# openMVG/openMVG

Hardware: AMD Instinct MI355X
Metric: descriptor pairs/s (brute-force L2 2-NN + ratio matching) (higher is better)
Workload: dtype i8 (int32 accumulate); 1 GPU; 1000 images x 2000 SIFT-like uint8x128 descriptors, exhaustive pairs (499500 image pairs, 499500 on rank 0), ratio 0.8; parallelism=pair-sharded x1, no collective

## Files before the change

### openmvg_amd/csrc/mvgx_match.hip

```cpp
#include <hip/hip_runtime.h>

#include <algorithm>
#include <atomic>
#include <climits>
#include <condition_variable>
#include <cstdint>
#include <cstdlib>
#include <cstring>
#include <functional>
#include <mutex>
#include <string>
#include <thread>
#include <vector>

#include "mvgx_buffers.h"
#include "mvgx_common.h"
#include "mvgx_match_batch.h"

namespace {

using mvgx::DevBuf;
using mvgx::PinnedBuf;
using mvgx::set_error;

// ... 703 lines not shown
  stage_window_glds_asm(buf, gtiles, grconst, wave, lane);
#endif
}

__device__ __forceinline__ void fold_window16(const int (&TW)[4], int (&TP)[4], int& Q1, int& Q2, int& Qg, int win) {
  const int v = max(max3i(TW[0], TW[1], TW[2]), TW[3]);
#pragma unroll
  for (int c = 0; c < 4; ++c) TP[c] = max(TP[c], TW[c]);
  Qg = v > Q1 ? win : Qg;
  Q2 = med3i(Q1, v, Q2);
  asm volatile("" : "+v"(Q1));
  Q1 = max(Q1, v);
}

struct UnitBlock { uint32_t pair, tileJ0, row0, nJ; };
__device__ __forceinline__ UnitBlock unit_block(const uint4& a, const uint4& b, uint32_t n) {
  const bool inA = n < b.z;
  return UnitBlock{inA ? a.x : b.x, inA ? a.y : b.y, (inA ? a.z + n : n - b.z) * 16u, inA ? a.w : b.w};
}

#define MVGX_FINISH16_MED3(N, INB, VALID)                                                                                                 \
  {                                                                                                                                       \
    int p1 = kNegInit, p2 = kNegInit, pc = 0;                                                \
    _Pragma("unroll") for (int c = 0; c < 4; ++c) {                                                                                       \
      const int v = TP[N][c];                                                                                                             \
      pc = v > p1 ? c : pc;                                                                                                               \
      p2 = med3i(p1, v, p2);                                                                                                              \
      p1 = max(p1, v);                                                                                                                    \
    }                                                                                                                                     \
                          \
    int W1 = 2 * p1 - par, V2 = max(2 * p2 - par, 2 * Q2[N] - par);                                                                       \
    int code = (4 * (pc >> 1) + 2 * (g4 >> 1) + (pc & 1)) | (par << 3) | (Qg[N] << 4);    \
                                                  \
    _Pragma("unroll") for (int x = 16; x <= 32; x <<= 1) {                                                                                \
      const int o1 = __shfl_xor(W1, x), o2 = __shfl_xor(V2, x), oc = __shfl_xor(code, x);                                                 \
      const bool mine = W1 > o1;                                                                                                          \
      V2 = mine ? max(V2, o1) : max(o2, W1);                                                                                              \
      code = mine ? code : oc;                                                                                                            \
      W1 = mine ? W1 : o1;                                                                                                                \
    }                                                                                                                                     \
    const UnitBlock ub = unit_block(wa, wb, (uint32_t)(N));                  \
    const uint32_t q = ub.row0 + (uint32_t)(lane & 15);                                                                                   \
    if (lane < 16 && (INB)) {                                                                                                             \
      const int nq = qn[N];                                                                                                               \
      const int d0 = nq - W1, d1ub = nq - V2;                                                                                             \
      const bool cand = (VALID) && (__int2float_rn(d0) < __fmul_rn(p.ratio_sq, __int2float_rn(d1ub)));                                    \
      const size_t o = (size_t)ub.pair * p.qstride + q;                                                                                   \
      p.best[o] = cand ? (uint32_t)code : kNoMatch;                                                                                       \
      if (cand) p.cd[o] = make_int2(d0, d1ub);                                                                                            \
    }                                                                                                                                     \
  }

__global__ __launch_bounds__(256, 2) void l2_filter16_kernel(MatchParams p) {
  extern __shared__ __attribute__((aligned(16))) char smem[];

  const int lane = threadIdx.x & 63;
  const int wave = __builtin_amdgcn_readfirstlane(threadIdx.x >> 6);
  const int g4 = lane >> 4, par = g4 & 1;

  const uint32_t w = xcd_remap(blockIdx.x, gridDim.x);
  const uint4* rec = p.work8 + (size_t)kRecQuads * w;
  const uint4 wsh = rec[0], wa = rec[1 + 2 * wave], wb = rec[2 + 2 * wave];
  const uint32_t tileI0 = wsh.x;
  const int ntI = (int)wsh.y;
  const int nwin = (ntI + kWinTiles - 1) / kWinTiles;

  const int lane_chunk = ((lane >> 5) * 64 + ((lane >> 4) & 1) * 32 + (lane & 15)) * 16;
  v4i b[kNB16][2];
  {
#pragma unroll
    for (int n = 0; n < kNB16; ++n) {
      const UnitBlock ub = unit_block(wa, wb, (uint32_t)n);
      const int8_t* qsrc = p.qtiles + ((size_t)(ub.tileJ0 + (ub.row0 >> 5)) * kTileBytes + ((ub.row0 >> 4) & 1u) * 256u) + lane_chunk;
#pragma unroll
      for (int ks = 0; ks < 2; ++ks) b[n][ks] = *reinterpret_cast<const v4i*>(qsrc + ks * 2048);
    }
  }

  const int8_t* gI = p.tiles + (size_t)tileI0 * kTileBytes;
  const int* gC = p.cinit + (size_t)tileI0 * kTileRows;

  int qn[kNB16];
#pragma unroll
  for (int n = 0; n < kNB16; ++n) {
    const UnitBlock ub = unit_block(wa, wb, (uint32_t)n);
    const uint32_t q = ub.row0 + (uint32_t)(lane & 15);
    qn[n] = (lane < 16 && q < ub.nJ) ? p.qtnorm[(size_t)ub.tileJ0 * kTileRows + q] : 0;
  }

  int TP[kNB16][4];
  int TW[kNB16][4];
  int Q1[kNB16], Q2[kNB16], Qg[kNB16];
#pragma unroll
  for (int n = 0; n < kNB16; ++n) {
#pragma unroll
    for (int c = 0; c < 4; ++c) TP[n][c] = kNegInit;
    Q1[n] = kNegInit; Q2[n] = kNegInit; Qg[n] = 0;
  }

  const unsigned voff16 = (unsigned)(lane * 16 + wave * 1024), voff4 = (unsigned)(lane * 4 + wave * 256);
  stage_window16(smem, gI, gC, voff16, voff4, wave, lane);
#pragma unroll
  for (int n = 0; n < kNB16; ++n) {
#pragma unroll
    for (int ks = 0; ks < 2; ++ks) asm volatile("" : "+v"(b[n][ks]));
    asm volatile("" : "+v"(qn[n]));
  }

  for (int win = 0; win < nwin; ++win) {
    asm volatile("s_waitcnt vmcnt(0)" ::: "memory");
    __syncthreads();
    char* buf = smem + (win & 1) * kStageBytes;
    char* nbuf = smem + ((win + 1) & 1) * kStageBytes;
    if (win + 1 < nwin)
      stage_window16(nbuf, gI + (size_t)(win + 1) * kWinTiles * kTileBytes, gC + (win + 1) * kWinRows, voff16, voff4, wave, lane);

    const int nt = min(kWinTiles, ntI - win * kWinTiles);
    const char* wb = buf + lane_chunk;
    const char* wc = buf + kWinTiles * kTileBytes + g4 * 16;
    v4i accA[4], accB[4];

#define MVGX_BLOCK16(A, CV, AN, CN, BLK, LD, NEXT_OFF, NEXT_COFF, EPI_B, MIX_B, EPI_A)                      \
  {                                                                                                         \
    MVGX_GROUP16(accA, 0, A, CV)                                                                            \
    if (LD) {                                                                                               \
      AN[0] = *reinterpret_cast<const v4i*>(wb + (NEXT_OFF));                                               \
      AN[1] = *reinterpret_cast<const v4i*>(wb + (NEXT_OFF) + 2048);                                        \
    }                                                                                                       \
    EPI_B(accB, 4, 1 - (BLK))                                                                               \
    MIX_B((LD) ? 2 : 0)                                                                                     \
    MVGX_GROUP16(accB, 4, A, CV)                                                                            \
    if (LD) CN = *reinterpret_cast<const v4i*>(wc + (NEXT_COFF));                                           \
    EPI_A(accA, 0, BLK)                                                                                     \
    MVGX_MIX16((LD) ? 1 : 0)                                                                                \
  }
#define MVGX_TILE16(T)                                                                                                                       \
  MVGX_BLOCK16(a0, c0, a1, c1, 0, true, (T) * kTileBytes + 256, (T) * (kTileRows * 4) + 64, MVGX_EPI16, MVGX_MIX16, MVGX_EPI16)              \
  MVGX_BLOCK16(a1, c1, a0, c0, 1, true, ((T) + 1) * kTileBytes, ((T) + 1) * (kTileRows * 4), MVGX_EPI16, MVGX_MIX16, MVGX_EPI16)                \
  MVGX_TILE16_END
#define MVGX_TILE16_END __builtin_amdgcn_sched_barrier(0);
    v4i a0[2], a1[2], c0, c1;
    a0[0] = *reinterpret_cast<const v4i*>(wb);
    a0[1] = *reinterpret_cast<const v4i*>(wb + 2048);
    c0 = *reinterpret_cast<const v4i*>(wc);
    __builtin_amdgcn_s_setprio(3);
    if (nt == kWinTiles) {
      MVGX_BLOCK16(a0, c0, a1, c1, 0, true, 256, 64, MVGX_EPI16_NONE, MVGX_MIX16_NOEPI, MVGX_EPI16_FIRST)
      MVGX_BLOCK16(a1, c1, a0, c0, 1, true, kTileBytes, kTileRows * 4, MVGX_EPI16_FIRST, MVGX_MIX16, MVGX_EPI16_FIRST)
      MVGX_TILE16_END
      MVGX_BLOCK16(a0, c0, a1, c1, 0, true, kTileBytes + 256, kTileRows * 4 + 64, MVGX_EPI16_FIRST, MVGX_MIX16, MVGX_EPI16)
      MVGX_BLOCK16(a1, c1, a0, c0, 1, true, 2 * kTileBytes, 2 * (kTileRows * 4), MVGX_EPI16, MVGX_MIX16, MVGX_EPI16)
      MVGX_TILE16_END
      MVGX_TILE16(2) MVGX_TILE16(3) MVGX_TILE16(4) MVGX_TILE16(5) MVGX_TILE16(6)
      MVGX_BLOCK16(a0, c0, a1, c1, 0, true, 7 * kTileBytes + 256, 7 * (kTileRows * 4) + 64, MVGX_EPI16, MVGX_MIX16, MVGX_EPI16)
      MVGX_BLOCK16(a1, c1, a0, c0, 1, false, 0, 0, MVGX_EPI16, MVGX_MIX16, MVGX_EPI16)
    } else {
#pragma unroll
      for (int n = 4; n < kNB16; ++n) { TW[n][2] = kNegInit; TW[n][3] = kNegInit; }
      const int t1 = min(1, nt - 1);
      MVGX_BLOCK16(a0, c0, a1, c1, 0, true, 256, 64, MVGX_EPI16_NONE, MVGX_MIX16_NOEPI, MVGX_EPI16_FIRST)
      MVGX_BLOCK16(a1, c1, a0, c0, 1, true, t1 * kTileBytes, t1 * (kTileRows * 4), MVGX_EPI16_FIRST, MVGX_MIX16, MVGX_EPI16_FIRST)
      for (int t = 1; t < nt; ++t) {
        const int tn = min(t + 1, nt - 1);
        MVGX_BLOCK16(a0, c0, a1, c1, 0, true, t * kTileBytes + 256, t * (kTileRows * 4) + 64, MVGX_EPI16, MVGX_MIX16, MVGX_EPI16)
        MVGX_BLOCK16(a1, c1, a0, c0, 1, true, tn * kTileBytes, tn * (kTileRows * 4), MVGX_EPI16, MVGX_MIX16, MVGX_EPI16)
      }
    }
    MVGX_EPI16(accB, 4, 1)
    __builtin_amdgcn_s_setprio(0);
#undef MVGX_TILE16
#undef MVGX_TILE16_END
#undef MVGX_BLOCK16
#pragma unroll
    for (int n = 0; n < kNB16; ++n) fold_window16(TW[n], TP[n], Q1[n], Q2[n], Qg[n], win);
  }

#pragma unroll
  for (int n = 0; n < kNB16; ++n) MVGX_FINISH16_MED3(n, q < ub.nJ, true)
}

constexpr int kNQh = 2;
constexpr int kNBh = 2 * kNQh;
constexpr int kBlockQTilesH = kWaves * kNQh;
__global__ __launch_bounds__(256, 3) void l2_filter16h_kernel(MatchParams p) {
  extern __shared__ __attribute__((aligned(16))) char smem[];

  const int lane = threadIdx.x & 63;
  const int wave = __builtin_amdgcn_readfirstlane(threadIdx.x >> 6);
  const int g4 = lane >> 4, par = g4 & 1;

  const uint32_t w = xcd_remap(blockIdx.x, gridDim.x);
  const uint4 wr0 = p.work8h[2 * (size_t)w], wr1 = p.work8h[2 * (size_t)w + 1];
  const uint32_t pair = wr0.x;
  const uint32_t tileI0 = wr0.z, tileJ0 = wr0.w;
  const uint32_t ntJpad = wr1.y;
  const int ntI = (int)wr1.x;
  const int nhalf = (ntI + kHalfTiles - 1) / kHalfTiles;
  const uint32_t qt0 = wr0.y + (uint32_t)wave * kNQh;

  const int lane_chunk = ((lane >> 5) * 64 + ((lane >> 4) & 1) * 32 + (lane & 15)) * 16;
  v4i b[kNBh][2];
  {
    const int8_t* qsrc = p.tiles + (size_t)(tileJ0 + qt0) * kTileBytes + lane_chunk;
#pragma unroll
    for (int n = 0; n < kNBh; ++n)
#pragma unroll
      for (int ks = 0; ks < 2; ++ks) b[n][ks] = *reinterpret_cast<const v4i*>(qsrc + (n >> 1) * kTileBytes + (n & 1) * 256 + ks * 2048);
  }
  const int8_t* gI = p.tiles + (size_t)tileI0 * kTileBytes;
  const int* gC = p.cinit + (size_t)tileI0 * kTileRows;

  uint32_t qperm[kNBh];
  int qn[kNBh];
#pragma unroll
  for (int n = 0; n < kNBh; ++n) {
    const bool inb = lane < 16 && qt0 + (uint32_t)(n >> 1) < ntJpad;
    const size_t qs = (size_t)tileJ0 * kTileRows + (qt0 + (uint32_t)(n >> 1)) * kTileRows + (uint32_t)(n & 1) * 16 + (uint32_t)(lane & 15);
    qperm[n] = inb ? p.perm[qs] : kNoMatch;
    qn[n] = inb ? p.qnorm[qs] : 0;
  }

  int TP[kNBh][4], TW[kNBh][4], Q1[kNBh], Q2[kNBh], Qg[kNBh];
#pragma unroll
  for (int n = 0; n < kNBh; ++n) {
#pragma unroll
    for (int c = 0; c < 4; ++c) { TP[n][c] = kNegInit; TW[n][c] = kNegInit; }
    Q1[n] = kNegInit; Q2[n] = kNegInit; Qg[n] = 0;
  }

  stage_half_glds_asm(smem, gI, gC, wave, lane);
#pragma unroll
  for (int n = 0; n < kNBh; ++n) {
#pragma unroll
    for (int ks = 0; ks < 2; ++ks) asm volatile("" : "+v"(b[n][ks]));
    asm volatile("" : "+v"(qperm[n]), "+v"(qn[n]));
  }

  for (int hw = 0; hw < nhalf; ++hw) {
    asm volatile("s_waitcnt vmcnt(0)" ::: "memory");
    __syncthreads();
    char* buf = smem + (hw & 1) * kHalfStageBytes;
    char* nbuf = smem + ((hw + 1) & 1) * kHalfStageBytes;
    if (hw + 1 < nhalf)
      stage_half_glds_asm(nbuf, gI + (size_t)(hw + 1) * kHalfTiles * kTileBytes, gC + (hw + 1) * kHalfTiles * kTileRows, wave, lane);

    const int nt = min(kHalfTiles, ntI - hw * kHalfTiles);
    const char* wb = buf + lane_chunk;
    const char* wc = buf + kHalfTiles * kTileBytes + g4 * 16;
    v4i accA[4], accB[4];
#pragma unroll
    for (int i = 0; i < 4; ++i) accB[i] = v4i{kNegInit, kNegInit, kNegInit, kNegInit};
    v4i a0[2], a1[2], c0, c1;
    a0[0] = *reinterpret_cast<const v4i*>(wb);
    a0[1] = *reinterpret_cast<const v4i*>(wb + 2048);
    c0 = *reinterpret_cast<const v4i*>(wc);
    for (int t = 0; t < nt; ++t) {
      const int tn = min(t + 1, nt - 1);
      MVGX_GROUP16(accA, 0, a0, c0)
      a1[0] = *reinterpret_cast<const v4i*>(wb + t * kTileBytes + 256);
      a1[1] = *reinterpret_cast<const v4i*>(wb + t * kTileBytes + 256 + 2048);
      c1 = *reinterpret_cast<const v4i*>(wc + t * (kTileRows * 4) + 64);
      MVGX_EPI16(accB, 0, 1)
      MVGX_MIX16(3)
      MVGX_GROUP16(accB, 0, a1, c1)
      a0[0] = *reinterpret_cast<const v4i*>(wb + tn * kTileBytes);
      a0[1] = *reinterpret_cast<const v4i*>(wb + tn * kTileBytes + 2048);
      c0 = *reinterpret_cast<const v4i*>(wc + tn * (kTileRows * 4));
      MVGX_EPI16(accA, 0, 0)
      MVGX_MIX16(3)
    }
    MVGX_EPI16(accB, 0, 1)
    if ((hw & 1) || hw + 1 == nhalf) {
#pragma unroll
      for (int n = 0; n < kNBh; ++n) fold_window<4>(TW[n], TP[n], Q1[n], Q2[n], Qg[n], hw >> 1);
    }
  }

#pragma unroll
  for (int n = 0; n < kNBh; ++n) MVGX_FINISH16(n, qt0 + (uint32_t)(n >> 1) < ntJpad, qperm[n] != kNoMatch)
}
#undef MVGX_FINISH16
#undef MVGX_GROUP16
#undef MVGX_EPI16
#undef MVGX_MIX16

__device__ __forceinline__ int sum8_dpp(int v) {
  v += __builtin_amdgcn_update_dpp(0, v, 0xB1, 0xF, 0xF, true);
  v += __builtin_amdgcn_update_dpp(0, v, 0x4E, 0xF, 0xF, true);
  v += __builtin_amdgcn_update_dpp(0, v, 0x141, 0xF, 0xF, true);
  return v;
}
__device__ __forceinline__ int min16_dpp(int v) {
  v = min(v, __builtin_amdgcn_update_dpp(INT_MAX, v, 0xB1, 0xF, 0xF, false));
  v = min(v, __builtin_amdgcn_update_dpp(INT_MAX, v, 0x4E, 0xF, 0xF, false));
  v = min(v, __builtin_amdgcn_update_dpp(INT_MAX, v, 0x141, 0xF, 0xF, false));
  v = min(v, __builtin_amdgcn_update_dpp(INT_MAX, v, 0x140, 0xF, 0xF, false));
  return v;
}

template <bool kWaveUnits>
__global__ __launch_bounds__(256) void l2_verify_kernel(MatchParams p) {
  const int lane = threadIdx.x & 63;
  const int wave = threadIdx.x >> 6;
  uint32_t pair, qt0, I, tileI0, tileJ0, qend;
  uint4 wa = make_uint4(0, 0, 0, 0), wb = wa;
  const uint8_t *rowsJA = nullptr, *rowsJB = nullptr;
  if constexpr (kWaveUnits) {
    const uint4* rec = p.work8 + (size_t)kRecQuads * blockIdx.x;
    const int wu = __builtin_amdgcn_readfirstlane(wave);
    wa = rec[1 + 2 * wu]; wb = rec[2 + 2 * wu];
    tileI0 = rec[0].x;
    const uint2 ijA = p.pairs[wa.x], ijB = p.pairs[wb.x];
    I = ijA.x;
    rowsJA = p.rows_u8 + p.img_row_off[ijA.y] * kDim;
    rowsJB = p.rows_u8 + p.img_row_off[ijB.y] * kDim;
    pair = 0; qt0 = 0; tileJ0 = 0; qend = 0;
  } else {
    const uint2 wk = p.work[blockIdx.x];
    const uint2 ij = p.pairs[wk.x];
    pair = wk.x; qt0 = wk.y + (uint32_t)wave * kNQ;
    I = ij.x;
    tileI0 = p.img_tile_off[I]; tileJ0 = p.img_tile_off[ij.y];
    qend = (p.img_tile_off[ij.y + 1] - tileJ0) * kTileRows;
  }
  const uint32_t nEvenI = p.img_neven[I], nOddI = p.img_n[I] - nEvenI;
  const int l16 = lane & 15, sub = lane >> 4;
  uint32_t accepted = 0, acceptedB = 0;
  for (int part = 0; part < 2; ++part) {
    const uint32_t q0 = qt0 * kTileRows + (uint32_t)part * 64;
    uint32_t q = q0 + lane, qpair = pair;
    bool inb = q < qend;
    if constexpr (kWaveUnits) {
      const UnitBlock ub = unit_block(wa, wb, (uint32_t)(part * 4 + sub));
      q = ub.row0 + (uint32_t)l16; qpair = ub.pair; inb = q < ub.nJ;
    }
    const uint32_t code = inb ? p.best[(size_t)qpair * p.qstride + q] : kNoMatch;
    unsigned long long todo = __ballot(code != kNoMatch);
    while (todo) {
      unsigned long long m = todo;
      for (int i = 0; i < sub; ++i) m &= m - 1;
      const bool active = m != 0;
      const int src = active ? __builtin_ctzll(m) : 0;
      for (int i = 0; i < 4; ++i) todo &= todo - 1;
      const uint32_t cc = (uint32_t)__shfl((int)code, src);
      uint32_t qs = q0 + (uint32_t)src, cpair = pair;
      bool inA = true;
      const uint8_t* rowsJ = nullptr;
      if constexpr (kWaveUnits) {
        const uint32_t cb = (uint32_t)(part * 4 + (src >> 4));
        const UnitBlock ub = unit_block(wa, wb, cb);
        qs = ub.row0 + (uint32_t)(src & 15); cpair = ub.pair; inA = cb < wb.z;
        rowsJ = inA ? rowsJA : rowsJB;
      }
      const int s1 = cc & 7, hw = (cc >> 3) & 1, g1 = (int)(cc >> 4);
      const int piece = l16 & 7, rsel = l16 >> 3;
      const int mrow = slot_row(2 * s1 + rsel, hw);
      const size_t slot0 = (size_t)tileI0 * kTileRows + (active ? (size_t)g1 * kWinTiles * kTileRows + mrow : 0);
      const size_t slotQ = (size_t)tileJ0 * kTileRows + (active ? qs : 0);
      const size_t o = (size_t)cpair * p.qstride + (active ? qs : 0);
      const uint32_t tt = (uint32_t)g1 * kWinTiles + (uint32_t)piece;
      const size_t slotI = active ? slot0 + (size_t)piece * kTileRows : slot0;
      const bool valid = active && (tt * 16u + (uint32_t)(2 * s1 + rsel)) < (hw ? nOddI : nEvenI);
      int4 va[8];
#pragma unroll
      for (int c = 0; c < 8; ++c)
        va[c] = *reinterpret_cast<const int4*>(p.rows_slot + (slot0 + (active ? (size_t)c * kTileRows : 0)) * kDim + piece * 16);
      int4 vb;
      if constexpr (kWaveUnits) {
        vb = *reinterpret_cast<const int4*>(rowsJ + (size_t)(active ? qs : 0) * kDim + piece * 16);
        vb.x ^= (int)0x80808080u; vb.y ^= (int)0x80808080u; vb.z ^= (int)0x80808080u; vb.w ^= (int)0x80808080u;
      } else {
        vb = *reinterpret_cast<const int4*>(p.rows_slot + slotQ * kDim + piece * 16);
      }
      const int2 f = p.cd[o];
      const int f_d0 = f.x, f_d1 = f.y;
      int nb = __builtin_amdgcn_sdot4(vb.x, vb.x, 0, false);
      nb = __builtin_amdgcn_sdot4(vb.y, vb.y, nb, false);
      nb = __builtin_amdgcn_sdot4(vb.z, vb.z, nb, false);
      nb = __builtin_amdgcn_sdot4(vb.w, vb.w, nb, false);
      nb = sum8_dpp(nb);
      int dot = 0, na = 0;
#pragma unroll
      for (int c = 0; c < 8; ++c) {
        int part = __builtin_amdgcn_sdot4(va[c].x, vb.x, 0, false);
        part = __builtin_amdgcn_sdot4(va[c].y, vb.y, part, false);
        part = __builtin_amdgcn_sdot4(va[c].z, vb.z, part, false);
        part = __builtin_amdgcn_sdot4(va[c].w, vb.w, part, false);
        part = sum8_dpp(part);
        dot = (c == piece) ? part : dot;
        int sq = __builtin_amdgcn_sdot4(va[c].x, va[c].x, 0, false);
        sq = __builtin_amdgcn_sdot4(va[c].y, va[c].y, sq, false);
        sq = __builtin_amdgcn_sdot4(va[c].z, va[c].z, sq, false);
        sq = __builtin_amdgcn_sdot4(va[c].w, va[c].w, sq, false);
        sq = sum8_dpp(sq);
        na = (c == piece) ? sq : na;
      }
      const int d = valid ? na + nb - 2 * dot : INT_MAX;
      const int key = min16_dpp(valid ? ((d << 4) | l16) : INT_MAX);
      const int wl = key & 15, dbest = key >> 4;
      const int second = min16_dpp((l16 == wl) ? INT_MAX : d);
      bool ok = false;
      if (active && l16 == wl) {
        if (key == INT_MAX || dbest != f_d0) atomicAdd(p.errflag, 1u);
        const int d1 = min(f_d1, second);
        ok = __int2float_rn(dbest) < __fmul_rn(p.ratio_sq, __int2float_rn(d1));
        p.best[o] = ok ? p.perm[slotI] : kNoMatch;
      }
      accepted += (uint32_t)__popcll(__ballot(ok && inA));
      if constexpr (kWaveUnits) acceptedB += (uint32_t)__popcll(__ballot(ok && !inA));
    }
  }
  if constexpr (kWaveUnits) {
    if (lane == 0 && accepted) atomicAdd(&p.count[wa.x], accepted);
    if (lane == 0 && acceptedB) atomicAdd(&p.count[wb.x], acceptedB);
  } else {
    if (lane == 0 && accepted) atomicAdd(&p.count[pair], accepted);
  }
}

__global__ __launch_bounds__(256) void count_candidates_kernel(const uint32_t* __restrict__ best, size_t n,
                                                               uint32_t* __restrict__ counter) {
  __shared__ uint32_t s_sum;
  if (threadIdx.x == 0) s_sum = 0;
  __syncthreads();
  uint32_t c = 0;
  const size_t base = (size_t)blockIdx.x * 16384;
  for (int k = 0; k < 64; ++k) {
    const size_t i = base + (size_t)k * 256 + threadIdx.x;
    if (i < n && best[i] != kNoMatch) ++c;
  }
  const unsigned long long m = __ballot(c != 0);
  (void)m;
  for (int off = 32; off > 0; off >>= 1) c += __shfl_down(c, off);
  if ((threadIdx.x & 63) == 0 && c) atomicAdd(&s_sum, c);
  __syncthreads();
  if (threadIdx.x == 0 && s_sum) atomicAdd(counter, s_sum);
}

__global__ __launch_bounds__(256) void count_candidates_units_kernel(MatchParams p, uint32_t* __restrict__ counter) {
  __shared__ uint32_t s_sum;
  if (threadIdx.x == 0) s_sum = 0;
  __syncthreads();
  const int lane = threadIdx.x & 63, wave = threadIdx.x >> 6;
  const uint4* rec = p.work8 + (size_t)kRecQuads * blockIdx.x;
  const uint4 wa = rec[1 + 2 * wave], wb = rec[2 + 2 * wave];
  uint32_t c = 0;
  for (int part = 0; part < 2; ++part) {
    const UnitBlock ub = unit_block(wa, wb, (uint32_t)(part * 4 + (lane >> 4)));
    const uint32_t q = ub.row0 + (uint32_t)(lane & 15);
    const bool cand = q < ub.nJ && p.best[(size_t)ub.pair * p.qstride + q] != kNoMatch;
    c += (uint32_t)__popcll(__ballot(cand));
  }
  if (lane == 0 && c) atomicAdd(&s_sum, c);
  __syncthreads();
  if (threadIdx.x == 0 && s_sum) atomicAdd(counter, s_sum);
}

__global__ __launch_bounds__(256) void l2_top2_ratio_naive_kernel(MatchParams p) {
  const uint2 wk = p.work[blockIdx.x];
  const uint2 ij = p.pairs[wk.x];
  const uint32_t I = ij.x, J = ij.y;
  const uint32_t nI = p.img_n[I], nJ = p.img_n[J];
  const uint8_t* rowsI = p.rows_u8 + p.img_row_off[I] * kDim;
  const uint8_t* rowsJ = p.rows_u8 + p.img_row_off[J] * kDim;
  for (uint32_t q = wk.y * kTileRows + threadIdx.x; q < min(nJ, (wk.y + kBlockQTiles) * kTileRows);
       q += blockDim.x) {
    uint32_t qv[32];
#pragma unroll
    for (int k = 0; k < 32; ++k) qv[k] = reinterpret_cast<const uint32_t*>(rowsJ + (size_t)q * kDim)[k];
    int d0 = INT_MAX, d1 = INT_MAX;
    uint32_t i0 = 0;
    for (uint32_t i = 0; i < nI; ++i) {
      const uint32_t* dbr = reinterpret_cast<const uint32_t*>(rowsI + (size_t)i * kDim);
      int d = 0;
#pragma unroll
      for (int k = 0; k < 32; ++k) {
        const uint32_t x = qv[k], y = dbr[k];
#pragma unroll
        for (int bb = 0; bb < 4; ++bb) {
          const int df = (int)((x >> (8 * bb)) & 0xFF) - (int)((y >> (8 * bb)) & 0xFF);
          d += df * df;
        }
      }
      if (d < d0) { d1 = d0; d0 = d; i0 = i; }
      else if (d < d1) { d1 = d; }
    }
    const bool ok = __int2float_rn(d0) < __fmul_rn(p.ratio_sq, __int2float_rn(d1));
    p.best[(size_t)wk.x * p.qstride + p.rowpos[p.img_row_off[J] + q]] = ok ? i0 : kNoMatch;
    if (ok) atomicAdd(&p.count[wk.x], 1u);
  }
}


}

#ifndef MVGX_MATCH_RECORD_ORDER
#define MVGX_MATCH_RECORD_ORDER 1
#endif

struct mvgx_match_ctx {
  int device = 0;
  hipStream_t stream = nullptr;
  hipEvent_t ev_total0 = nullptr, ev_total1 = nullptr;
  int variant = 4;
  int filter_shape = 16;
  int stage = 3;
  int profile = 0;
  int64_t batch_pairs = 1 << 15;
  int64_t batch_ramp = 1024;
  int record_order = MVGX_MATCH_RECORD_ORDER;
  int record_chunk_tiles = mvgx_records::kOrderChunkTiles;
  std::vector<uint32_t> h_rec_tmp, h_rec_count;
  int keep_host_results = 1;
  int overlap = 1;
  int verify_alone = 0;
  int debug_filter = 0;
  int stream_hold = 0;
  int pinned_stream = 1;
  uint32_t n_images = 0;
  uint32_t total_tiles = 0;
  uint32_t max_tiles_pad = 0;
  uint32_t qstride = 0;
  std::vector<uint32_t> h_n, h_tile_off, h_ntiles;
  std::vector<uint32_t> h_qtile_off;
  std::vector<uint64_t> h_row_off;
  DevBuf<uint8_t> d_rows;
  bool rows_owned = true;
  const uint8_t* d_rows_view = nullptr;
  DevBuf<int8_t> d_tiles, d_rows_slot, d_qtiles;
  DevBuf<int> d_rconst, d_cinit, d_qnorm, d_rownorm, d_qtnorm;
  DevBuf<uint64_t> d_row_off;
  DevBuf<uint32_t> d_tile_off, d_qtile_off, d_n, d_ntiles, d_perm, d_rowpos, d_neven, d_err;
  struct Slot {
    hipStream_t stream = nullptr;
    hipEvent_t ev_scan = nullptr;
    hipEvent_t ev_filter = nullptr;
    DevBuf<uint2> d_pairs, d_work, d_ij;
    DevBuf<uint4> d_work8, d_work8h;
    DevBuf<uint32_t> d_best, d_count, d_offsets;
    DevBuf<int2> d_cd;
    PinnedBuf<uint2> hp_pairs, hp_work;
    PinnedBuf<uint4> hp_work8, hp_work8h;
    PinnedBuf<uint32_t> hp_offsets;
    uint64_t p0 = 0;
    uint32_t nb = 0, cap = 0;
    hipEvent_t ev_copy = nullptr;
    PinnedBuf<uint32_t> hp_ij[2];
    std::vector<uint32_t> h_off_out[2];
    int out_set = 0;
    uint64_t out_p0 = 0;
    uint32_t out_nb = 0;
  } slot[2];
  struct Results {
    std::vector<uint64_t> offsets;
    PinnedBuf<uint32_t> ij;
    size_t ij_n = 0;
  } results[2];
  int cur = 0;
  int double_buffer = 0;
  std::vector<hipEvent_t> ev_pool;
  std::vector<mvgx_match_ctx*> children;
};

namespace {

enum WorkList { kListItems16 = 0, kListItems8h = 1, kListRecords = 2 };
using MatchKernel = void (*)(MatchParams);
struct KernelForm {
  MatchKernel filter;
  uint32_t lds_bytes;
  WorkList list;
  bool dense_slots;
  MatchKernel verify;
  WorkList verify_list;
  bool count_units;
  bool reads(WorkList l) const { return list == l || (verify && verify_list == l); }
};

KernelForm form_for(int variant, int filter_shape, int stage, int debug_filter) {
  constexpr uint32_t kTwoWindows = 2 * kStageBytes;
  auto exact = [](MatchKernel k, uint32_t lds) { return KernelForm{k, lds, kListItems16, false, nullptr, kListItems16, false}; };
  auto filter32 = [](MatchKernel k) { return KernelForm{k, kTwoWindows, kListItems16, false, &l2_verify_kernel<false>, kListItems16, false}; };
  if (variant == 0) return exact(&l2_top2_ratio_naive_kernel, 0);
  if (variant == 1) return exact(&l2_top2_ratio_kernel<kStageRegs>, kTwoWindows);
  if (variant == 2) return exact(&l2_top2_ratio_kernel<kStageGlds>, kTwoWindows);
  if (variant == 3) return exact(&l2_top2_ratio_kernel<kStageGldsAsm>, kTwoWindows);
  if (filter_shape == 16 && stage == 3 && !debug_filter)
    return KernelForm{&l2_filter16_kernel, kTwoWindows, kListRecords, true, &l2_verify_kernel<true>, kListRecords, true};
  if (filter_shape == 17 && stage == 3 && !debug_filter)
    return KernelForm{&l2_filter16h_kernel, 2 * kHalfStageBytes, kListItems8h, false, &l2_verify_kernel<false>, kListItems16, false};
  if (stage == 1) return filter32(&l2_filter_kernel<kStageRegs>);
  if (stage == 2) return filter32(&l2_filter_kernel<kStageGlds>);
  if (debug_filter == 8) return filter32(&l2_filter_kernel<kStageGldsAsm, kEpiPerChain>);
  if (debug_filter == 16) return filter32(&l2_filter_kernel<kStageGldsAsm, kEpiFoldOneCv>);
  return filter32(&l2_filter_kernel<kStageGldsAsm>);
}
KernelForm resolve_form(const mvgx_match_ctx* c) { return form_for(c->variant, c->filter_shape, c->stage, c->debug_filter); }

bool pair_has_work(const mvgx_match_ctx* c, uint32_t I, uint32_t J) { return mvgx_records::pair_has_work(c->h_n.data(), I, J); }

uint32_t build_items16(const mvgx_match_ctx* c, const uint32_t* ij, uint32_t nb, uint2* out) {
  uint32_t n = 0;
  for (uint32_t k = 0; k < nb; ++k) {
    const uint32_t I = ij[2 * k], J = ij[2 * k + 1];
    if (!pair_has_work(c, I, J)) continue;
    for (uint32_t qt = 0; qt < c->h_ntiles[J]; qt += kBlockQTiles) out[n++] = make_uint2(k, qt);
  }
  return n;
}
uint32_t build_items8h(const mvgx_match_ctx* c, const uint32_t* ij, uint32_t nb, uint4* out) {
  uint32_t n = 0;
  for (uint32_t k = 0; k < nb; ++k) {
    const uint32_t I = ij[2 * k], J = ij[2 * k + 1];
    if (!pair_has_work(c, I, J)) continue;
    for (uint32_t qt = 0; qt < c->h_ntiles[J]; qt += kBlockQTilesH) {
      out[2 * n] = make_uint4(k, qt, c->h_tile_off[I], c->h_tile_off[J]);
      out[2 * n + 1] = make_uint4(c->h_ntiles[I], c->h_tile_off[J + 1] - c->h_tile_off[J], 0, 0);
      ++n;
    }
  }
  return n;
}
uint32_t build_records(const mvgx_match_ctx* c, const uint32_t* ij, uint32_t nb, uint4* out) {
  const mvgx_records::ImageTables im{c->h_n.data(), c->h_tile_off.data(), c->h_ntiles.data(), c->h_qtile_off.data()};
  return mvgx_records::build_block_records(im, ij, nb, reinterpret_cast<uint32_t*>(out));
}

template <typename T>
int upload_list(DevBuf<T>& d, const PinnedBuf<T>& h, size_t n, hipStream_t stream, size_t reserve = 0) {
  const int rc = d.ensure(std::max<size_t>(std::max(n, reserve), 1));
  if (rc) return rc;
  if (n) MVGX_HIP(hipMemcpyAsync(d.p, h.p, n * sizeof(T), hipMemcpyHostToDevice, stream));
  return MVGX_OK;
}

int prep_regions(mvgx_match_ctx* c) {
  const uint32_t n_images = c->n_images;
  c->h_tile_off.assign(n_images + 1, 0);
  c->h_row_off.assign(n_images + 1, 0);
  c->h_ntiles.assign(n_images + 1, 0);
  c->h_qtile_off.assign(n_images + 1, 0);
  uint32_t max_n = 0;
  for (uint32_t k = 0; k < n_images; ++k) {
    c->h_row_off[k + 1] = c->h_row_off[k] + c->h_n[k];
    c->h_qtile_off[k + 1] = c->h_qtile_off[k] + (c->h_n[k] + kTileRows - 1) / kTileRows;
    max_n = std::max(max_n, c->h_n[k]);
  }
  const uint64_t total_rows = c->h_row_off[n_images];
  int rc;
  if ((rc = c->d_row_off.ensure(n_images + 1))) return rc;
  if ((rc = c->d_tile_off.ensure(n_images + 1))) return rc;
  if ((rc = c->d_qtile_off.ensure(n_images + 1))) return rc;
  if ((rc = c->d_n.ensure(n_images + 1))) return rc;
  if ((rc = c->d_ntiles.ensure(n_images + 1))) return rc;
  if ((rc = c->d_neven.ensure(n_images + 1))) return rc;
  if ((rc = c->d_err.ensure(2))) return rc;
  if ((rc = c->d_rownorm.ensure(std::max<uint64_t>(total_rows, 1)))) return rc;
  if ((rc = c->d_rowpos.ensure(std::max<uint64_t>(total_rows, 1)))) return rc;
  MVGX_HIP(hipMemcpyAsync(c->d_row_off.p, c->h_row_off.data(), (n_images + 1) * sizeof(uint64_t),
                          hipMemcpyHostToDevice, c->stream));
  MVGX_HIP(hipMemcpyAsync(c->d_n.p, c->h_n.data(), n_images * sizeof(uint32_t), hipMemcpyHostToDevice, c->stream));
  MVGX_HIP(hipMemsetAsync(c->d_neven.p, 0, (n_images + 1) * sizeof(uint32_t), c->stream));
  MVGX_HIP(hipMemsetAsync(c->d_err.p, 0, 2 * sizeof(uint32_t), c->stream));
  std::vector<uint32_t> h_even(n_images + 1, 0);
  if (total_rows > 0) {
    dim3 grid((max_n + 255) / 256, n_images);
    hipLaunchKernelGGL(row_norms_kernel, grid, dim3(256), 0, c->stream, c->d_rows_view, c->d_row_off.p, c->d_n.p,
                       c->d_rownorm.p, c->d_neven.p);
    MVGX_HIP(hipGetLastError());
    MVGX_HIP(hipMemcpyAsync(h_even.data(), c->d_neven.p, n_images * sizeof(uint32_t), hipMemcpyDeviceToHost, c->stream));
  }
  MVGX_HIP(hipStreamSynchronize(c->stream));
  uint32_t max_pad = 0;
  for (uint32_t k = 0; k < n_images; ++k) {
    const uint32_t ne = h_even[k], no = c->h_n[k] - h_even[k];
    const uint32_t nt = (std::max(ne, no) + 15) / 16;
    const uint32_t pad = (nt + kWinTiles - 1) / kWinTiles * kWinTiles;
    c->h_ntiles[k] = nt;
    c->h_tile_off[k + 1] = c->h_tile_off[k] + pad;
    max_pad = std::max(max_pad, pad);
  }
  c->total_tiles = c->h_tile_off[n_images];
  c->max_tiles_pad = max_pad;
  c->qstride = max_pad * kTileRows;
  const size_t alloc_tiles = (size_t)c->total_tiles + kTailTiles;
  const size_t alloc_slots = alloc_tiles * kTileRows;
  if ((rc = c->d_tiles.ensure(alloc_tiles * kTileBytes))) return rc;
  if ((rc = c->d_rows_slot.ensure(alloc_tiles * kTileBytes))) return rc;
  if ((rc = c->d_rconst.ensure(alloc_slots))) return rc;
  if ((rc = c->d_cinit.ensure(alloc_slots))) return rc;
  if ((rc = c->d_qnorm.ensure(alloc_slots))) return rc;
  if ((rc = c->d_perm.ensure(alloc_slots))) return rc;
  const size_t total_qtiles = c->h_qtile_off[n_images];
  if ((rc = c->d_qtiles.ensure((total_qtiles + kTailTiles) * kTileBytes))) return rc;
  if ((rc = c->d_qtnorm.ensure((total_qtiles + kTailTiles) * kTileRows))) return rc;
  MVGX_HIP(hipMemcpyAsync(c->d_qtile_off.p, c->h_qtile_off.data(), (n_images + 1) * sizeof(uint32_t), hipMemcpyHostToDevice, c->stream));
  MVGX_HIP(hipMemsetAsync(c->d_qtiles.p + total_qtiles * kTileBytes, 0, (size_t)kTailTiles * kTileBytes, c->stream));
  MVGX_HIP(hipMemsetAsync(c->d_qtnorm.p + total_qtiles * kTileRows, 0, (size_t)kTailTiles * kTileRows * sizeof(int), c->stream));
  MVGX_HIP(hipMemcpyAsync(c->d_tile_off.p, c->h_tile_off.data(), (n_images + 1) * sizeof(uint32_t),
                          hipMemcpyHostToDevice, c->stream));
  MVGX_HIP(hipMemcpyAsync(c->d_ntiles.p, c->h_ntiles.data(), (n_images + 1) * sizeof(uint32_t),
                          hipMemcpyHostToDevice, c->stream));
  const int fill_grid = (int)((alloc_slots + 255) / 256);
  hipLaunchKernelGGL(fill_i32_kernel, dim3(fill_grid), dim3(256), 0, c->stream, c->d_rconst.p, alloc_slots, kRPad);
  hipLaunchKernelGGL(fill_i32_kernel, dim3(fill_grid), dim3(256), 0, c->stream, c->d_cinit.p, alloc_slots, kCPad);
  hipLaunchKernelGGL(fill_i32_kernel, dim3(fill_grid), dim3(256), 0, c->stream, c->d_qnorm.p, alloc_slots, 0);
  hipLaunchKernelGGL(fill_i32_kernel, dim3(fill_grid), dim3(256), 0, c->stream, reinterpret_cast<int*>(c->d_perm.p),
                     alloc_slots, (int)kNoMatch);
  MVGX_HIP(hipGetLastError());
  MVGX_HIP(hipMemsetAsync(c->d_tiles.p + (size_t)c->total_tiles * kTileBytes, 0, (size_t)kTailTiles * kTileBytes,
                          c->stream));
  if (total_rows > 0 && max_pad > 0) {
    hipLaunchKernelGGL(assign_slots_kernel, dim3(n_images), dim3(1024), 0, c->stream, c->d_row_off.p, c->d_tile_off.p,
                       c->d_n.p, c->d_rownorm.p, c->d_rowpos.p, c->d_perm.p, c->d_rconst.p, c->d_cinit.p, c->d_qnorm.p);
    MVGX_HIP(hipGetLastError());
    dim3 grid(max_pad, n_images);
    hipLaunchKernelGGL(build_tiles_kernel, grid, dim3(256), 0, c->stream, c->d_rows_view, c->d_row_off.p,
                       c->d_tile_off.p, c->d_perm.p, c->d_tiles.p, c->d_rows_slot.p);
    MVGX_HIP(hipGetLastError());
    dim3 qgrid((max_n + kTileRows - 1) / kTileRows, n_images);
    hipLaunchKernelGGL(build_qtiles_kernel, qgrid, dim3(256), 0, c->stream, c->d_rows_view, c->d_row_off.p, c->d_qtile_off.p, c->d_n.p,
// ... 636 lines not shown
```

Before: 10780 billion descriptor pairs/s.

## Specialise wave-unit L2 verify kernel with compacted candidates and transposed reduction

Splits the wave-unit path of the L2 verify kernel into its own specialisation. Candidate rows from both parts are compacted with a lane scatter so each iteration processes four real candidates. The per-chunk dot and norm sums are combined through a butterfly transpose reduction, which replaces eight separate 8-lane DPP reductions per candidate with three DPP steps. The specialisation also uses 32-bit offsets, scalar base pointers and inline asm hints. The fallback scatter path without MVGX_GLDS_SBASE is a slow 64-iteration shuffle loop, and the 32-bit offset arithmetic could overflow on large buffers.

Measured after the change: 10970 billion descriptor pairs/s, median of 6. 1.8% higher.

```diff
diff --git a/openmvg_amd/csrc/mvgx_match.hip b/openmvg_amd/csrc/mvgx_match.hip
--- a/openmvg_amd/csrc/mvgx_match.hip
+++ b/openmvg_amd/csrc/mvgx_match.hip
@@ -1029,39 +1029,19 @@
 __global__ __launch_bounds__(256) void l2_verify_kernel(MatchParams p) {
   const int lane = threadIdx.x & 63;
   const int wave = threadIdx.x >> 6;
-  uint32_t pair, qt0, I, tileI0, tileJ0, qend;
-  uint4 wa = make_uint4(0, 0, 0, 0), wb = wa;
-  const uint8_t *rowsJA = nullptr, *rowsJB = nullptr;
-  if constexpr (kWaveUnits) {
-    const uint4* rec = p.work8 + (size_t)kRecQuads * blockIdx.x;
-    const int wu = __builtin_amdgcn_readfirstlane(wave);
-    wa = rec[1 + 2 * wu]; wb = rec[2 + 2 * wu];
-    tileI0 = rec[0].x;
-    const uint2 ijA = p.pairs[wa.x], ijB = p.pairs[wb.x];
-    I = ijA.x;
-    rowsJA = p.rows_u8 + p.img_row_off[ijA.y] * kDim;
-    rowsJB = p.rows_u8 + p.img_row_off[ijB.y] * kDim;
-    pair = 0; qt0 = 0; tileJ0 = 0; qend = 0;
-  } else {
-    const uint2 wk = p.work[blockIdx.x];
-    const uint2 ij = p.pairs[wk.x];
-    pair = wk.x; qt0 = wk.y + (uint32_t)wave * kNQ;
-    I = ij.x;
-    tileI0 = p.img_tile_off[I]; tileJ0 = p.img_tile_off[ij.y];
-    qend = (p.img_tile_off[ij.y + 1] - tileJ0) * kTileRows;
-  }
+  static_assert(!kWaveUnits, "the form after l2_filter16_kernel is the specialisation below");
+  const uint2 wk = p.work[blockIdx.x];
+  const uint2 ij = p.pairs[wk.x];
+  const uint32_t pair = wk.x, qt0 = wk.y + (uint32_t)wave * kNQ, I = ij.x;
+  const uint32_t tileI0 = p.img_tile_off[I], tileJ0 = p.img_tile_off[ij.y];
+  const uint32_t qend = (p.img_tile_off[ij.y + 1] - tileJ0) * kTileRows;
   const uint32_t nEvenI = p.img_neven[I], nOddI = p.img_n[I] - nEvenI;
   const int l16 = lane & 15, sub = lane >> 4;
-  uint32_t accepted = 0, acceptedB = 0;
+  uint32_t accepted = 0;
   for (int part = 0; part < 2; ++part) {
     const uint32_t q0 = qt0 * kTileRows + (uint32_t)part * 64;
-    uint32_t q = q0 + lane, qpair = pair;
-    bool inb = q < qend;
-    if constexpr (kWaveUnits) {
-      const UnitBlock ub = unit_block(wa, wb, (uint32_t)(part * 4 + sub));
-      q = ub.row0 + (uint32_t)l16; qpair = ub.pair; inb = q < ub.nJ;
-    }
-    const uint32_t code = inb ? p.best[(size_t)qpair * p.qstride + q] : kNoMatch;
+    const uint32_t q = q0 + lane;
+    const uint32_t code = q < qend ? p.best[(size_t)pair * p.qstride + q] : kNoMatch;
     unsigned long long todo = __ballot(code != kNoMatch);
     while (todo) {
       unsigned long long m = todo;
@@ -1070,21 +1050,13 @@
       const int src = active ? __builtin_ctzll(m) : 0;
       for (int i = 0; i < 4; ++i) todo &= todo - 1;
       const uint32_t cc = (uint32_t)__shfl((int)code, src);
-      uint32_t qs = q0 + (uint32_t)src, cpair = pair;
-      bool inA = true;
-      const uint8_t* rowsJ = nullptr;
-      if constexpr (kWaveUnits) {
-        const uint32_t cb = (uint32_t)(part * 4 + (src >> 4));
-        const UnitBlock ub = unit_block(wa, wb, cb);
-        qs = ub.row0 + (uint32_t)(src & 15); cpair = ub.pair; inA = cb < wb.z;
-        rowsJ = inA ? rowsJA : rowsJB;
-      }
+      const uint32_t qs = q0 + (uint32_t)src;
       const int s1 = cc & 7, hw = (cc >> 3) & 1, g1 = (int)(cc >> 4);
       const int piece = l16 & 7, rsel = l16 >> 3;
       const int mrow = slot_row(2 * s1 + rsel, hw);
       const size_t slot0 = (size_t)tileI0 * kTileRows + (active ? (size_t)g1 * kWinTiles * kTileRows + mrow : 0);
       const size_t slotQ = (size_t)tileJ0 * kTileRows + (active ? qs : 0);
-      const size_t o = (size_t)cpair * p.qstride + (active ? qs : 0);
+      const size_t o = (size_t)pair * p.qstride + (active ? qs : 0);
       const uint32_t tt = (uint32_t)g1 * kWinTiles + (uint32_t)piece;
       const size_t slotI = active ? slot0 + (size_t)piece * kTileRows : slot0;
       const bool valid = active && (tt * 16u + (uint32_t)(2 * s1 + rsel)) < (hw ? nOddI : nEvenI);
@@ -1092,13 +1064,7 @@
 #pragma unroll
       for (int c = 0; c < 8; ++c)
         va[c] = *reinterpret_cast<const int4*>(p.rows_slot + (slot0 + (active ? (size_t)c * kTileRows : 0)) * kDim + piece * 16);
-      int4 vb;
-      if constexpr (kWaveUnits) {
-        vb = *reinterpret_cast<const int4*>(rowsJ + (size_t)(active ? qs : 0) * kDim + piece * 16);
-        vb.x ^= (int)0x80808080u; vb.y ^= (int)0x80808080u; vb.z ^= (int)0x80808080u; vb.w ^= (int)0x80808080u;
-      } else {
-        vb = *reinterpret_cast<const int4*>(p.rows_slot + slotQ * kDim + piece * 16);
-      }
+      const int4 vb = *reinterpret_cast<const int4*>(p.rows_slot + slotQ * kDim + piece * 16);
       const int2 f = p.cd[o];
       const int f_d0 = f.x, f_d1 = f.y;
       int nb = __builtin_amdgcn_sdot4(vb.x, vb.x, 0, false);
@@ -1133,17 +1099,167 @@
         ok = __int2float_rn(dbest) < __fmul_rn(p.ratio_sq, __int2float_rn(d1));
         p.best[o] = ok ? p.perm[slotI] : kNoMatch;
       }
-      accepted += (uint32_t)__popcll(__ballot(ok && inA));
-      if constexpr (kWaveUnits) acceptedB += (uint32_t)__popcll(__ballot(ok && !inA));
-    }
-  }
-  if constexpr (kWaveUnits) {
-    if (lane == 0 && accepted) atomicAdd(&p.count[wa.x], accepted);
-    if (lane == 0 && acceptedB) atomicAdd(&p.count[wb.x], acceptedB);
-  } else {
-    if (lane == 0 && accepted) atomicAdd(&p.count[pair], accepted);
-  }
-}
+      accepted += (uint32_t)__popcll(__ballot(ok));
+    }
+  }
+  if (lane == 0 && accepted) atomicAdd(&p.count[pair], accepted);
+}
+
+__device__ __forceinline__ int lane_scatter(int v, int dst) {
+#ifdef MVGX_GLDS_SBASE
+  return __builtin_amdgcn_ds_permute(dst << 2, v);
+#else
+  const int lane = threadIdx.x & 63;
+  int out = 0;
+  for (int l = 0; l < 64; ++l) {
+    const int d = __shfl(dst, l), x = __shfl(v, l);
+    out = d == lane ? x : out;
+  }
+  return out;
+#endif
+}
+__device__ __forceinline__ int lane_gather(int v, int src) {
+#ifdef MVGX_GLDS_SBASE
+  return __builtin_amdgcn_ds_bpermute(src << 2, v);
+#else
+  return __shfl(v, src & 63);
+#endif
+}
+__device__ __forceinline__ int dot4_first(int a, int b) {
+#ifdef MVGX_GLDS_SBASE
+  int r;
+  asm("v_dot4_i32_i8 %0, %1, %2, 0" : "=v"(r) : "v"(a), "v"(b));
+  return r;
+#else
+  return __builtin_amdgcn_sdot4(a, b, 0, false);
+#endif
+}
+#define MVGX_TSUM(KEEP_LO, KEEP_HI, CTRL) \
+  ((upper ? (KEEP_HI) : (KEEP_LO)) + __builtin_amdgcn_update_dpp(0, upper ? (KEEP_LO) : (KEEP_HI), (CTRL), 0xF, 0xF, true))
+
+template <>
+__global__ __launch_bounds__(256) void l2_verify_kernel<true>(MatchParams p) {
+  const int lane = threadIdx.x & 63;
+  const int wu = __builtin_amdgcn_readfirstlane(threadIdx.x >> 6);
+  const int l16 = lane & 15, sub = lane >> 4;
+  const int piece = l16 & 7, rsel = l16 >> 3;
+  const uint4* rec = p.work8 + (size_t)kRecQuads * blockIdx.x;
+  const uint4 wsh = rec[0], wa = rec[1 + 2 * wu], wb = rec[2 + 2 * wu];
+  const uint2 ijA = p.pairs[wa.x], ijB = p.pairs[wb.x];
+  const uint32_t rowA = (uint32_t)p.img_row_off[ijA.y], rowB = (uint32_t)p.img_row_off[ijB.y];
+  const uint32_t nEvenI = p.img_neven[ijA.x], nOddI = p.img_n[ijA.x] - nEvenI;
+  const uint32_t baseA = wa.x * p.qstride, baseB = wb.x * p.qstride;
+
+  uint32_t code[2], row[2];
+  bool segA[2];
+#pragma unroll
+  for (int part = 0; part < 2; ++part) {
+    const uint32_t blk = (uint32_t)(part * 4 + sub);
+    const UnitBlock ub = unit_block(wa, wb, blk);
+    row[part] = ub.row0 + (uint32_t)l16;
+    segA[part] = blk < wb.z;
+    const bool inb = row[part] < ub.nJ;
+    const uint32_t w = *reinterpret_cast<const uint32_t*>(reinterpret_cast<const char*>(p.best) +
+                                                          (inb ? (ub.pair * p.qstride + row[part]) * 4u : 0u));
+    code[part] = inb ? w : kNoMatch;
+  }
+  const unsigned long long m0 = __ballot(code[0] != kNoMatch), m1 = __ballot(code[1] != kNoMatch);
+  const int n0 = __popcll(m0), total = n0 + __popcll(m1);
+  if (total == 0) return;
+
+  const unsigned long long below = (1ull << lane) - 1ull;
+  int PX[2], PY[2];
+#pragma unroll
+  for (int part = 0; part < 2; ++part) {
+    const uint32_t cc = code[part];
+    const int s1 = cc & 7, hw = (cc >> 3) & 1, g1 = (int)(cc >> 4);
+    const int slotbase = g1 * (kWinTiles * kTileRows) + slot_row(2 * s1, hw);
+    const int left = (int)(hw ? nOddI : nEvenI) - (g1 * (kWinTiles * 16) + 2 * s1);
+    const int X = (slotbase << 9) | (min(max(left, 0), 128) << 1) | (segA[part] ? 1 : 0);
+    const bool cand = cc != kNoMatch;
+    const int r = __popcll((part ? m1 : m0) & below);
+    const int first = part ? n0 : 0, behind = part ? total : n0;
+    const int dst = (cand ? first + r : behind + (lane - r)) & 63;
+    PX[part] = lane_scatter(X, dst);
+    PY[part] = lane_scatter((int)row[part], dst);
+  }
+  const int D0X = lane < n0 ? PX[0] : PX[1], D0Y = lane < n0 ? PY[0] : PY[1];
+
+  const char __attribute__((address_space(1)))* rowsI[8];
+#pragma unroll
+  for (int c = 0; c < 8; ++c) {
+    rowsI[c] = (const char __attribute__((address_space(1)))*)(p.rows_slot + ((size_t)wsh.x + c) * kTileRows * kDim);
+    asm volatile("" : "+s"(rowsI[c]));
+  }
+  const uint32_t* permI = p.perm + (size_t)wsh.x * kTileRows;
+  const uint32_t lane_bytes = (uint32_t)(rsel * kDim + piece * 16);
+  const uint32_t lane_slot = (uint32_t)(rsel + piece * kTileRows);
+  const int lane_rank = piece * 16 + rsel;
+  uint32_t accepted = 0, acceptedB = 0;
+  for (int k = 0; 4 * k < total; ++k) {
+    const int want = 4 * k + sub;
+    const bool active = want < total;
+    const int src = min(want, total - 1);
+    const int X = lane_gather(k < 16 ? D0X : PX[1], src), Y = lane_gather(k < 16 ? D0Y : PY[1], src);
+    const uint32_t slotbase = (uint32_t)X >> 9, qs = (uint32_t)Y;
+    const bool inA = X & 1;
+    const bool valid = lane_rank < ((X >> 1) & 0xFF);
+    const uint32_t voff = slotbase * kDim + lane_bytes;
+    v4i va[8];
+#pragma unroll
+    for (int c = 0; c < 8; ++c) va[c] = *(const v4i __attribute__((address_space(1)))*)(rowsI[c] + voff);
+    const uint32_t grow = (inA ? rowA : rowB) + qs;
+    int4 vb = *reinterpret_cast<const int4*>(p.rows_u8 + (size_t)grow * kDim + piece * 16);
+    vb.x ^= (int)0x80808080u; vb.y ^= (int)0x80808080u; vb.z ^= (int)0x80808080u; vb.w ^= (int)0x80808080u;
+    const uint32_t o = (inA ? baseA : baseB) + qs;
+    const int2 f = *reinterpret_cast<const int2*>(reinterpret_cast<const char*>(p.cd) + o * 8u);
+    int f_d0 = f.x, f_d1 = f.y;
+    int nb = dot4_first(vb.x, vb.x);
+    nb = __builtin_amdgcn_sdot4(vb.y, vb.y, nb, false);
+    nb = __builtin_amdgcn_sdot4(vb.z, vb.z, nb, false);
+    nb = __builtin_amdgcn_sdot4(vb.w, vb.w, nb, false);
+    nb = sum8_dpp(nb);
+    int part[8];
+#pragma unroll
+    for (int c = 0; c < 8; ++c) {
+      int ab = dot4_first(va[c].x, vb.x), aa = dot4_first(va[c].x, va[c].x);
+      ab = __builtin_amdgcn_sdot4(va[c].y, vb.y, ab, false); aa = __builtin_amdgcn_sdot4(va[c].y, va[c].y, aa, false);
+      ab = __builtin_amdgcn_sdot4(va[c].z, vb.z, ab, false); aa = __builtin_amdgcn_sdot4(va[c].z, va[c].z, aa, false);
+      ab = __builtin_amdgcn_sdot4(va[c].w, vb.w, ab, false); aa = __builtin_amdgcn_sdot4(va[c].w, va[c].w, aa, false);
+      part[c] = aa - 2 * ab;
+    }
+    int own_row;
+    {
+      int t[4], u[2];
+      bool upper = piece & 4;
+#pragma unroll
+      for (int i = 0; i < 4; ++i) t[i] = MVGX_TSUM(part[i], part[4 + i], 0x141);
+      upper = piece & 2;
+#pragma unroll
+      for (int i = 0; i < 2; ++i) u[i] = MVGX_TSUM(t[i], t[2 + i], 0x4E);
+      upper = piece & 1;
+      own_row = MVGX_TSUM(u[0], u[1], 0xB1);
+    }
+    const int d = valid ? own_row + nb : INT_MAX;
+    asm volatile("" : "+v"(f_d0), "+v"(f_d1));
+    const int key = min16_dpp(valid ? ((d << 4) | l16) : INT_MAX);
+    const int wl = key & 15, dbest = key >> 4;
+    const int second = min16_dpp((l16 == wl) ? INT_MAX : d);
+    bool ok = false;
+    if (active && l16 == wl) {
+      if (key == INT_MAX || dbest != f_d0) atomicAdd(p.errflag, 1u);
+      const int d1 = min(f_d1, second);
+      ok = __int2float_rn(dbest) < __fmul_rn(p.ratio_sq, __int2float_rn(d1));
+      const uint32_t orig = *reinterpret_cast<const uint32_t*>(reinterpret_cast<const char*>(permI) + (slotbase + lane_slot) * 4u);
+      *reinterpret_cast<uint32_t*>(reinterpret_cast<char*>(p.best) + o * 4u) = ok ? orig : kNoMatch;
+    }
+    accepted += (uint32_t)__popcll(__ballot(ok && inA));
+    acceptedB += (uint32_t)__popcll(__ballot(ok && !inA));
+  }
+  if (lane == 0 && accepted) atomicAdd(&p.count[wa.x], accepted);
+  if (lane == 0 && acceptedB) atomicAdd(&p.count[wb.x], acceptedB);
+}
+#undef MVGX_TSUM
 
 __global__ __launch_bounds__(256) void count_candidates_kernel(const uint32_t* __restrict__ best, size_t n,
                                                                uint32_t* __restrict__ counter) {
```
